# ucsdmanorlab/PSSR2

Hardware: AMD Instinct MI355X
Metric: HR tiles/sec (512^2 4xSR) train (higher is better)
Workload: dtype bf16

## Files before the change

### include/pssr_mi355.h

```cpp
#ifndef PSSR_MI355_H
#define PSSR_MI355_H

#include <stdint.h>

#ifdef __cplusplus
extern "C" {
#endif

typedef void* pssr_stream_t;

enum { PSSR_F32 = 0, PSSR_BF16 = 1, PSSR_F16 = 2 };

enum {
    PSSR_OK = 0,
    PSSR_ERR_ARG = -1,
    PSSR_ERR_LAUNCH = -2,
    PSSR_ERR_UNSUPPORTED = -3
};

int pssr_abi_version(void);
const char* pssr_last_error(void);

int pssr_pack_conv_weight(const float* w_oihw, void* packed, int cout, int cin, int ks,
                          int ci_begin, int ci_count, int mode, const int32_t* n_perm,
// ... 178 lines not shown
int pssr_bilinear_down_u8(const uint8_t* hr, uint8_t* tmp, uint8_t* lr, int planes, int H, int W,
                          int h, int w, pssr_stream_t stream);
int pssr_u8_to_f32(const uint8_t* in, float* out, int64_t n, pssr_stream_t stream);
int pssr_crappify_gaussian(const float* in, float* out, int tiles, int64_t per_tile, float intensity,
                           float gain, float spread, uint64_t seed, uint64_t tile_offset,
                           const double* noise, int flags, const uint64_t* tile_counter,
                           pssr_stream_t stream);
int pssr_crappify_poisson(const float* in, float* out, int tiles, int64_t per_tile, float intensity,
                          float gain, float spread, uint64_t seed, uint64_t tile_offset, int flags,
                          const uint64_t* tile_counter, pssr_stream_t stream);
int pssr_crappify_poisson_samples(const float* in, const double* samples, float* out, int64_t n, double intensity,
                                  double gain, int flags, pssr_stream_t stream);
int pssr_counter_add(uint64_t* counter, uint64_t inc, pssr_stream_t stream);
int pssr_gaussian_blur(const float* in, float* tmp, float* out, int planes, int h, int w, float sigma,
                       float gain, int flags, pssr_stream_t stream);

int pssr_crappify_saltpepper(const float* in, float* out, int tiles, int64_t per_tile, float amount, float gain, float spread,
                             uint64_t seed, uint64_t tile_offset, int flags, const uint64_t* tile_counter, pssr_stream_t stream);
int pssr_gaussian_blur_tiles(const float* in, float* tmp, float* out, int tiles, int planes_per_tile, int h, int w, float sigma,
                             float spread, float gain, uint64_t seed, uint64_t tile_offset, int flags, const uint64_t* tile_counter,
                             pssr_stream_t stream);
typedef struct pssr_gather_item { const uint8_t* src; int sh, sw, rot, flip_axis; } pssr_gather_item;
int pssr_gen_pair_geometry_u8(const pssr_gather_item* items_dev, int n_items, uint8_t* out, int c, int res, pssr_stream_t stream);
typedef struct pssr_sheet_desc { const uint8_t* base; int frames, h, w, reserved; } pssr_sheet_desc;
typedef struct pssr_window_item { int sheet, frame0, y0, x0, rot, flip_axis; } pssr_window_item;
int pssr_gather_windows_u8(const pssr_sheet_desc* sheets_dev, int n_sheets, const pssr_window_item* items_dev, int n_items,
                           uint8_t* out, int c, int res, pssr_stream_t stream);


int pssr_input_plain(const float* x_nchw, void* out, int n, int c, int h, int w, int out_cs, float pre_scale, float pre_shift,
                     int dtype, pssr_stream_t stream);
int pssr_im2col_dil(const void* in, int in_cs, int in_co, int c, const float* scale, const float* shift, void* col, int cp,
                    int n, int h, int w, int dil, int dtype, pssr_stream_t stream);
int pssr_col2im_dil(const void* dcol, int cp, void* out, int out_cs, int out_co, int c, int n, int h, int w, int dil,
                    const void* y, int y_cs, int y_co, const float* scale, const float* shift, const float* mean,
                    const float* invstd, double* stats, int dtype, pssr_stream_t stream);
int pssr_channel_stats_nhwc(const void* x, int cs, int co, int c, int64_t npix, double* stats, int dtype, pssr_stream_t stream);
int pssr_sum_relu(const void* const* ins, const int* in_cs, const int* in_co, int n_in, void* out, int out_cs, int out_co,
                  int64_t npix, int c, int relu, int dtype, pssr_stream_t stream);
int pssr_relu_mask(const void* dout, int do_cs, int do_co, const void* out, int o_cs, int o_co, void* dz, int dz_cs, int dz_co,
                   int64_t npix, int c, int dtype, pssr_stream_t stream);
int pssr_affine_relu(const void* x, int cs, int co, const float* scale, const float* shift, void* out, int out_cs, int out_co,
                     int64_t npix, int c, int dtype, pssr_stream_t stream);
int pssr_maxpool_k(const void* in, int in_cs, int in_co, void* out, int out_cs, int out_co, int n, int h, int w, int c, int k,
                   int dtype, pssr_stream_t stream);
int pssr_maxpool_k_bwd(const void* act, int act_cs, int act_co, const void* dpool, int dp_cs, int dp_co, void* dx, int dx_cs,
// ... 127 lines not shown
```

### pssr2_amd/_lib.py

```python
from __future__ import annotations

import ctypes as C
import os
from pathlib import Path

_LIB_PATH = Path(__file__).resolve().parent / "libpssr_mi355.so"
_lib = None

F32, BF16, F16 = 0, 1, 2
PRO_NONE, PRO_BN_RELU, PRO_GELU = 0, 1, 2
EPI_STORE, EPI_TAIL, EPI_DGRAD_MASK, EPI_FINAL, EPI_DGRAD_GELU, EPI_HEADQ = 0, 1, 2, 3, 4, 5
FLAG_RELU, FLAG_STATS, FLAG_AFFINE, FLAG_HEADQ, FLAG_SHUF2, FLAG_SOLO = 1, 2, 4, 8, 16, 32

c_void_p, c_int, c_i64, c_float = C.c_void_p, C.c_int, C.c_int64, C.c_float


class ConvDesc(C.Structure):
    _fields_ = [
        ("dtype", C.c_int32), ("n", C.c_int32), ("h", C.c_int32), ("w", C.c_int32),
        ("in0", c_void_p), ("in0_cstride", C.c_int32), ("in0_coff", C.c_int32), ("cin0", C.c_int32), ("taps0", C.c_int32),
        ("w0", c_void_p),
        ("in1", c_void_p), ("in1_cstride", C.c_int32), ("in1_coff", C.c_int32), ("cin1", C.c_int32), ("taps1", C.c_int32),
        ("w1", c_void_p),
        ("prologue", C.c_int32), ("pro_scale", c_void_p), ("pro_shift", c_void_p),
# ... 58 lines not shown
                ("mode", C.c_int32), ("k_pad", C.c_int32), ("n_pad", C.c_int32), ("dtype", C.c_int32), ("center", C.c_int32)]


def lib():
    global _lib
    if _lib is None:
        if not _LIB_PATH.exists():
            raise RuntimeError(
                f"{_LIB_PATH} not found: build the HIP extension first (python -c 'import __graft_entry__ as g; g.build()' "
                "or make -C pssr2_amd/csrc). pssr2_amd has no CPU fallback.")
        import torch
        _lib = C.CDLL(str(_LIB_PATH))
        _lib.pssr_last_error.restype = C.c_char_p
        _lib.pssr_packed_weight_bytes.restype = C.c_int64
        _lib.pssr_conv2d_workspace_bytes.restype = C.c_int64
        _lib.pssr_gradhist_workspace_bytes.restype = C.c_int64
        _lib.pssr_noise_profile_workspace_bytes.restype = C.c_int64
        _lib.pssr_noise_profile_workspace_bytes.argtypes = [c_int, c_i64]
        for name in ("pssr_noise_profile_f32", "pssr_noise_profile_u8"):
            getattr(_lib, name).argtypes = [c_void_p, c_void_p, c_void_p, c_void_p, c_int, c_i64, c_void_p, c_i64, c_void_p]
        _lib.pssr_noise_profile_loss.argtypes = [c_void_p, c_void_p, c_void_p, c_void_p, c_int, c_i64, c_int, c_void_p, c_void_p, c_void_p,
                                                 c_void_p]
        _lib.pssr_gather_windows_u8.argtypes = [c_void_p, c_int, c_void_p, c_int, c_void_p, c_int, c_int, c_void_p]
    return _lib


def check(status: int, what: str):
    if status != 0:
        raise RuntimeError(f"{what} failed ({status}): {lib().pssr_last_error().decode()}")


def ptr(t):
    return None if t is None else c_void_p(t.data_ptr())


def stream_ptr():
    import torch
    return c_void_p(torch.cuda.current_stream().cuda_stream)
```

### pssr2_amd/csrc/crappify.hip

```cpp
#include "common.h"

namespace {

constexpr int PRECISION_BITS = 32 - 8 - 2;

struct Taps { int xmin, n; int k[40]; };
__device__ __forceinline__ void pil_taps(int xx, int in_size, int out_size, Taps& t) {
    const double scale = (double)in_size / (double)out_size;
    const double filterscale = scale < 1.0 ? 1.0 : scale;
    const double support = 1.0 * filterscale;
    const double center = (xx + 0.5) * scale;
    const double ss = 1.0 / filterscale;
    int xmin = (int)(center - support + 0.5);
    if (xmin < 0) xmin = 0;
    int xmax = (int)(center + support + 0.5);
    if (xmax > in_size) xmax = in_size;
    const int n = xmax - xmin;
    double w[40];
    double ww = 0.0;
    for (int x = 0; x < n && x < 40; ++x) {
        double a = (x + xmin - center + 0.5) * ss;
        if (a < 0.0) a = -a;
        const double v = a < 1.0 ? 1.0 - a : 0.0;
        w[x] = v; ww += v;
// ... 54 lines not shown
        }
        return make_uint4(c0, c1, c2, c3);
    }
};
__device__ __forceinline__ double u01(uint32_t hi, uint32_t lo) {
    const uint64_t v = (((uint64_t)hi << 32) | lo) >> 11;
    return ((double)v + 0.5) * (1.0 / 9007199254740992.0);
}
__device__ __forceinline__ double normal_from(const uint4& r) {
    const double u1 = u01(r.x, r.y), u2 = u01(r.z, r.w);
    return sqrt(-2.0 * log(u1)) * cos(6.283185307179586476925 * u2);
}
__device__ __forceinline__ double finish(double v, int flags) {
    if (flags & 2) v = rint(v);
    if (flags & 3) v = v < 0.0 ? 0.0 : (v > 255.0 ? 255.0 : v);
    return v;
}
__device__ __forceinline__ double tile_intensity(const Philox& ph, float intensity, float spread) {
    if (!(spread > 0.f)) return intensity;
    const double v = (double)intensity + (double)spread * normal_from(ph(~0ull, 7u));
    return v > 0.0 ? v : 0.0;
}

__global__ void gaussian_noise_kernel(const float* __restrict__ in, float* __restrict__ out, int tiles, long per_tile, float intensity,
                                      float gain, float spread, uint64_t seed, uint64_t tile_offset, const double* __restrict__ noise, int flags,
                                      const uint64_t* __restrict__ tile_counter) {
    if (tile_counter) tile_offset += tile_counter[0];
    const long total = (long)tiles * per_tile;
    for (long i = blockIdx.x * (long)blockDim.x + threadIdx.x; i < total; i += (long)gridDim.x * blockDim.x) {
        const long tile = i / per_tile, pix = i % per_tile;
        double nz;
        if (noise) nz = noise[i];
        else {
            const Philox ph(seed, tile_offset + tile);
            nz = (double)gain + tile_intensity(ph, intensity, spread) * normal_from(ph((uint64_t)pix, 0u));
        }
        out[i] = (float)finish((double)in[i] + nz, flags);
    }
}

__device__ double poisson_draw(const Philox& ph, uint64_t pix, double lam) {
    if (lam <= 0.0) return 0.0;
    uint32_t sub = 1;
    if (lam < 10.0) {
        const double enlam = exp(-lam);
        double prod = 1.0; long x = 0;
        for (int it = 0; it < 64; ++it) {
            const uint4 r = ph(pix, sub++);
            const double u[2] = {u01(r.x, r.y), u01(r.z, r.w)};
            for (int j = 0; j < 2; ++j) { prod *= u[j]; if (prod > enlam) ++x; else return (double)x; }
        }
        return (double)x;
    }
    const double slam = sqrt(lam), loglam = log(lam);
    const double b = 0.931 + 2.53 * slam, a = -0.059 + 0.02483 * b;
    const double invalpha = 1.1239 + 1.1328 / (b - 3.4), vr = 0.9277 - 3.6224 / (b - 2.0);
    for (int it = 0; it < 256; ++it) {
        const uint4 r = ph(pix, sub++);
        const double U = u01(r.x, r.y) - 0.5, V = u01(r.z, r.w);
        const double us = 0.5 - fabs(U);
        const double k = floor((2.0 * a / us + b) * U + lam + 0.43);
        if (us >= 0.07 && V <= vr) return k;
        if (k < 0.0 || (us < 0.013 && V > us)) continue;
        if (log(V) + log(invalpha) - log(a / (us * us) + b) <= -lam + k * loglam - lgamma(k + 1.0)) return k;
    }
    return floor(lam + 0.5);
}

__global__ void poisson_noise_kernel(const float* __restrict__ in, float* __restrict__ out, int tiles, long per_tile, float intensity,
                                     float gain, float spread, uint64_t seed, uint64_t tile_offset, int flags,
                                     const uint64_t* __restrict__ tile_counter) {
    if (tile_counter) tile_offset += tile_counter[0];
    const long total = (long)tiles * per_tile;
    for (long i = blockIdx.x * (long)blockDim.x + threadIdx.x; i < total; i += (long)gridDim.x * blockDim.x) {
        const long tile = i / per_tile, pix = i % per_tile;
        const Philox ph(seed, tile_offset + tile);
        const double x = (double)in[i];
        const double y = poisson_draw(ph, (uint64_t)pix, x > 0.0 ? x : 0.0);
        const double mixv = tile_intensity(ph, intensity, spread);
        out[i] = (float)finish(x * (1.0 - mixv) + y * mixv + (double)gain, flags);
    }
}

__global__ void poisson_samples_kernel(const float* __restrict__ in, const double* __restrict__ samples, float* __restrict__ out, long n,
                                       double intensity, double gain, int flags) {
    const float keep = (float)(1.0 - intensity);
    for (long i = blockIdx.x * (long)blockDim.x + threadIdx.x; i < n; i += (long)gridDim.x * blockDim.x) {
        const float t1 = __fmul_rn(in[i], keep);
        const double v = __dadd_rn(__dadd_rn((double)t1, __dmul_rn(samples[i], intensity)), gain);
        out[i] = (float)finish(v, flags);
    }
}

__global__ void blur_pass_kernel(const float* __restrict__ in, float* __restrict__ out, int planes, int h, int w, float sigma, int axis,
                                 float gain, int flags) {
    const int r = (int)(4.0f * sigma + 0.5f);
    const long total = (long)planes * h * w;
    for (long i = blockIdx.x * (long)blockDim.x + threadIdx.x; i < total; i += (long)gridDim.x * blockDim.x) {
        const int x = i % w, y = (i / w) % h;
        const long base = i - (long)y * w - x;
        double wsum = 0.0, acc = 0.0;
        for (int t = -r; t <= r; ++t) {
            const double wt = exp(-0.5 / ((double)sigma * sigma) * (double)t * t);
// ... 35 lines not shown
        const double sigma = tile_intensity(ph, intensity, spread);
        const int x = i % w, y = (i / w) % h;
        const long base = i - (long)y * w - x;
        double v = (double)in[i];
        if (sigma > 0.0) {
            const int r = (int)(4.0 * (double)(float)sigma + 0.5);
            double wsum = 0.0, acc = 0.0;
            for (int t = -r; t <= r; ++t) {
                const double wt = exp(-0.5 / (sigma * sigma) * (double)t * t);
                int yy = y, xx = x;
                if (axis == 0) { yy = y + t; yy = yy < 0 ? 0 : (yy >= h ? h - 1 : yy); }
                else { xx = x + t; xx = xx < 0 ? 0 : (xx >= w ? w - 1 : xx); }
                wsum += wt; acc += wt * (double)in[base + (long)yy * w + xx];
            }
            v = (double)(float)(acc / wsum);
        }
        if (axis == 1) v = finish((double)(float)v + (double)gain, flags);
        out[i] = (float)v;
    }
}

struct GatherItem { const uint8_t* src; int sh, sw, rot, flip_axis; };

__global__ void gen_pair_geometry_kernel(const GatherItem* __restrict__ items, uint8_t* __restrict__ out, int c, int res) {
    const GatherItem it = items[blockIdx.y];
    const long per_tile = (long)c * res * res;
    const int size = it.sh < it.sw ? (it.sh < res ? it.sh : res) : (it.sw < res ? it.sw : res);
    const bool exact = it.sh == res && it.sw == res;
    const int sx = exact ? 0 : (it.sh - size) / 2, sy = exact ? 0 : (it.sw - size) / 2;
    for (long i = blockIdx.x * (long)blockDim.x + threadIdx.x; i < per_tile; i += (long)gridDim.x * blockDim.x) {
        int ox = (int)(i % res), oy = (int)((i / res) % res), oc = (int)(i / ((long)res * res));
        if (it.flip_axis == 0) oc = c - 1 - oc;
        if (it.flip_axis == 1 || it.flip_axis == 3) oy = res - 1 - oy;
        if (it.flip_axis == 2 || it.flip_axis == 3) ox = res - 1 - ox;
        int py = oy, px = ox;
        if (it.rot) { py = ox; px = res - 1 - oy; }
        if (size > 1) {
            const int period = 2 * (size - 1);
            py %= period; px %= period;
            if (py >= size) py = period - py;
            if (px >= size) px = period - px;
        } else { py = 0; px = 0; }
        out[blockIdx.y * per_tile + i] = it.src[((long)oc * it.sh + sx + py) * it.sw + sy + px];
    }
}

static inline int grid1d(long total) { long b = (total + 255) / 256; return (int)(b < 8192 ? (b > 0 ? b : 1) : 8192); }

}

extern "C" {

int pssr_bilinear_down_u8(const uint8_t* hr, uint8_t* tmp, uint8_t* lr, int planes, int H, int W, int h, int w, pssr_stream_t s) {
    PSSR_CHECK(hr && tmp && lr && planes > 0 && H > 0 && W > 0 && h > 0 && w > 0, PSSR_ERR_ARG, "bilinear_down_u8: bad args");
    PSSR_CHECK(H >= h && W >= w && (double)W / w <= 19.0 && (double)H / h <= 19.0, PSSR_ERR_UNSUPPORTED, "bilinear_down_u8: reduction ratio must be in [1, 19]");
    long rows = (long)planes * H;
    const long row_groups = (rows + 15) / 16;
    hipLaunchKernelGGL(resample_h_kernel, dim3(cdiv(w, 64), (unsigned)(row_groups < 65535 ? row_groups : 65535)), dim3(64), 0, (hipStream_t)s, hr, tmp, planes, H, W, w);
    PSSR_LAUNCH_CHECK();
    hipLaunchKernelGGL(resample_v_kernel, dim3(cdiv(w, 128), h, planes < 1024 ? planes : 1024), dim3(128), 0, (hipStream_t)s, tmp, lr, planes, H, h, w);
    PSSR_LAUNCH_CHECK();
    return PSSR_OK;
}

int pssr_u8_to_f32(const uint8_t* in, float* out, int64_t n, pssr_stream_t s) {
    PSSR_CHECK(in && out && n > 0, PSSR_ERR_ARG, "u8_to_f32: bad args");
    hipLaunchKernelGGL(u8_to_f32_kernel, dim3(grid1d(n)), dim3(256), 0, (hipStream_t)s, in, out, (long)n);
    PSSR_LAUNCH_CHECK();
    return PSSR_OK;
// ... 58 lines not shown
                             float gain, uint64_t seed, uint64_t tile_offset, int flags, const uint64_t* tile_counter, pssr_stream_t s) {
    PSSR_CHECK(in && tmp && out && tiles > 0 && planes_per_tile > 0 && h > 0 && w > 0 && sigma >= 0.f && spread >= 0.f && flags >= 0 && flags <= 3,
               PSSR_ERR_ARG, "gaussian_blur_tiles: bad args");
    const long total = (long)tiles * planes_per_tile * h * w;
    hipLaunchKernelGGL(blur_pass_tiles_kernel, dim3(grid1d(total)), dim3(256), 0, (hipStream_t)s, in, tmp, tiles, planes_per_tile, h, w, sigma,
                       spread, seed, tile_offset, 0, 0.f, 0, tile_counter);
    PSSR_LAUNCH_CHECK();
    hipLaunchKernelGGL(blur_pass_tiles_kernel, dim3(grid1d(total)), dim3(256), 0, (hipStream_t)s, tmp, out, tiles, planes_per_tile, h, w, sigma,
                       spread, seed, tile_offset, 1, gain, flags, tile_counter);
    PSSR_LAUNCH_CHECK();
    return PSSR_OK;
}

int pssr_gen_pair_geometry_u8(const pssr_gather_item* items_dev, int n_items, uint8_t* out, int c, int res, pssr_stream_t s) {
    PSSR_CHECK(items_dev && out && n_items > 0 && n_items <= 65535 && c > 0 && res > 0, PSSR_ERR_ARG, "gen_pair_geometry: bad args");
    static_assert(sizeof(pssr_gather_item) == sizeof(GatherItem), "pssr_gather_item layout");
    const long per_tile = (long)c * res * res;
    long gx = (per_tile + 255) / 256; if (gx > 256) gx = 256;
    hipLaunchKernelGGL(gen_pair_geometry_kernel, dim3((unsigned)gx, n_items), dim3(256), 0, (hipStream_t)s, (const GatherItem*)items_dev, out, c, res);
    PSSR_LAUNCH_CHECK();
    return PSSR_OK;
}

}
```

### pssr2_amd/data.py

```python
from __future__ import annotations

import glob
import random
import warnings
from pathlib import Path

import numpy as np
import torch
from torch.utils.data import Dataset

from .crappifiers import Crappifier, Poisson
from .util import _force_list


def _square_crop(image, max_res):
    h, w = image.shape[-2:]
    if [h, w] == [max_res] * 2:
        return image
    size = min(h, w, max_res)
    sx, sy = (h - size) // 2, (w - size) // 2
    return image[:, sx:sx + size, sy:sy + size]


def _pad_image(image, res):
# ... 552 lines not shown
    def __repr__(self):
        return (f'PairedSlidingDataset from paths "{self.hr_path}" and "{self.lr_path}"\n{len(self.hr_files)} paired files with {len(self)} '
                f"total frame slices\nhigh-res: {self.hr_res}, low-res: {self.hr_res // self.lr_scale}")


def synthetic_em_tile(index, res=512, channels=1):
    rng = np.random.default_rng(1234 + index)
    out = []
    for _ in range(channels):
        white = rng.standard_normal((res, res))
        f = np.fft.rfft2(white)
        ky, kx = np.fft.fftfreq(res)[:, None], np.fft.rfftfreq(res)[None, :]
        smooth = np.fft.irfft2(f * np.exp(-2 * (np.pi * 3.0) ** 2 * (kx ** 2 + ky ** 2)), s=(res, res))
        smooth /= smooth.std() + 1e-12
        out.append(np.clip(128 + 48 * smooth + 8 * rng.standard_normal((res, res)), 0, 255).astype(np.uint8))
    return np.stack(out)


class DevicePairGenerator:

    def __init__(self, lr_scale=4, crappifier=Poisson(), seed=0, tile_counter=None):
        self.lr_scale, self.crappifier, self.seed = lr_scale, crappifier, seed
        self.tile_counter = tile_counter

    def _stage(self, x, spec, seed, tile_offset, flags):
        from . import ops
        kind, intensity, gain, spread = spec
        if kind == "gaussian":
            return ops.crappify_gaussian(x, intensity, gain, spread, seed, tile_offset, flags, tile_counter=self.tile_counter)
        if kind == "poisson":
            return ops.crappify_poisson(x, intensity, gain, spread, seed, tile_offset, flags, tile_counter=self.tile_counter)
        if kind == "blur":
            if spread > 0:
                return ops.gaussian_blur_tiles(x, intensity, spread, gain, seed, tile_offset, flags, tile_counter=self.tile_counter)
            return ops.gaussian_blur(x, intensity, gain, flags)
        if kind == "saltpepper":
            return ops.crappify_saltpepper(x, intensity, gain, spread, seed, tile_offset, flags, tile_counter=self.tile_counter)
        raise NotImplementedError(kind)

    def __call__(self, hr_u8: torch.Tensor, tile_offset: int = 0):
        from . import ops
        if not hr_u8.is_cuda or hr_u8.dtype != torch.uint8:
            raise RuntimeError("DevicePairGenerator needs a uint8 tensor on the MI355X")
        hr_u8 = hr_u8.contiguous()
        b, c, h, w = hr_u8.shape
        lr = ops.u8_to_f32(ops.bilinear_down_u8(hr_u8, h // self.lr_scale, w // self.lr_scale))
        cr = self.crappifier
        if cr is not None:
            spec = cr.device_spec()
            if isinstance(spec, list):
                clip = ops.CLIP if spec[0][0] == "clip" else 0
                stages = spec[1:]
                for i, st in enumerate(stages):
                    last = i == len(stages) - 1
                    lr = self._stage(lr, st, self.seed + 7919 * i, tile_offset, ops.ROUND_CLIP if last and clip else (clip if not last else 0))
                if not clip:
                    lr = self._stage(lr, ("gaussian", 0.0, 0.0, 0.0), 0, 0, ops.ROUND_CLIP)
            else:
                lr = self._stage(lr, spec, self.seed, tile_offset, ops.ROUND_CLIP)
        return ops.u8_to_f32(hr_u8), lr

    def from_stacks(self, stacks, hr_res, rotations=None, tile_offset: int = 0):
        from . import ops
        rotations = [False] * len(stacks) if rotations is None else rotations
        return self(ops.gen_pair_geometry_u8(stacks, rotations, hr_res), tile_offset)


def _gather_table(images, indices, rotations):
    import struct
    c, h, w = images.shape[1:]
    base, stride = images.data_ptr(), c * h * w
    buf = bytearray()
    for i, rot in zip(indices, rotations):
        axis = -1
        if rot:
            axis = 3 if isinstance(rot[1], (tuple, list)) else int(rot[1])
        buf += struct.pack("<Qiiii", base + int(i) * stride, h, w, int(bool(rot and rot[0])), axis)
    if not buf:
        return torch.zeros(0, 3, dtype=torch.int64, device=images.device)
    return torch.frombuffer(buf, dtype=torch.int64).view(-1, 3).to(images.device)


class DeviceTileDataset(Dataset):
# ... 23 lines not shown
        self.names = names if names is not None else [f"image{i}" for i in range(n)]
        self._val_set, self._val_key = set(self.val_idx), None
        self.tile_counter = torch.zeros(1, dtype=torch.int64, device=self.images.device)
        self.gen = DevicePairGenerator(self.lr_scale, crappifier, seed=seed, tile_counter=self.tile_counter)
        self._item_bytes = 24

    def __len__(self):
        return len(self.images)

    def _get_name(self, idx):
        return self.names[idx]

    def _draw_rotation(self, idx):
        key = (id(self.val_idx), len(self.val_idx))
        if key != self._val_key:
            self._val_set, self._val_key = set(self.val_idx), key
        if self.rotation and idx not in self._val_set:
            return [bool(random.getrandbits(1)), random.choice((1, 2, (1, 2)))]
        return False

    def draw_items(self, indices):
        return _gather_table(self.images, indices, [self._draw_rotation(int(i)) for i in indices])

    def device_batch(self, items):
        from . import _lib as L, ops
        b, c = items.shape[0], self.images.shape[1]
        res = self.hr_res // self.lr_scale if self.is_lr else self.hr_res
        out = torch.empty(b, c, res, res, dtype=torch.uint8, device=self.images.device)
        L.check(L.lib().pssr_gen_pair_geometry_u8(L.ptr(items), b, L.ptr(out), c, res, L.stream_ptr()), "pssr_gen_pair_geometry_u8")
        if self.is_lr:
            return ops.u8_to_f32(out)
        hr, lr = self.gen(out)
        ops.counter_add(self.tile_counter, b)
        return hr, lr

    def __getitem__(self, idx):
        if idx >= len(self):
            raise IndexError(f"Tried to retrieve invalid image. Index {idx} is not less than {len(self)} total image frame slices.")
        out = self.device_batch(self.draw_items([idx]))
        return out[0] if self.is_lr else (out[0][0], out[1][0])


class DevicePairedTileDataset(PairedArrayDataset):
    _keep_tensors = True

    def __init__(self, hr_images, lr_images, hr_res=512, lr_scale=4, n_frames=-1, val_split=1, rotation=True, split_seed=None,
                 transforms=None, names=None, device="cuda"):
        if transforms is not None:
            raise NotImplementedError("DevicePairedTileDataset applies no host transforms")
        super().__init__(hr_images, lr_images, hr_res, lr_scale, n_frames, val_split, rotation, split_seed, None, names)
        self.hr_images = torch.as_tensor(self.hr_images).to(device).contiguous()
        self.lr_images = torch.as_tensor(self.lr_images).to(device).contiguous()
        if not self.hr_images.is_cuda:
            raise RuntimeError("DevicePairedTileDataset keeps its images on an MI355X (HIP) device; there is no CPU fallback")
        del self.compact

    def draw_pair_items(self, indices, pp=False):
# ... 79 lines not shown
        self.sheets = self.bank.sheets
        del self.compact
        self.tile_counter = torch.zeros(1, dtype=torch.int64, device=self.bank.device)
        self.gen = DevicePairGenerator(self.lr_scale, crappifier, seed=seed, tile_counter=self.tile_counter)
        self._item_bytes = 24

    def draw_items(self, indices, pp=False):
        entries = []
        for idx in indices:
            idx = int(idx)
            self._check_idx(idx)
            image_idx, local = _get_image_idx(idx, self.slices, self.tiles)
            origin = _window_origin(self.sheets[image_idx], self.hr_res, self.stride, None if self.n_frames is None else self.depth,
                                    self.slices[image_idx], local, self.slide)
            self.bank.check(image_idx, *origin, self.depth, self.hr_res)
            entries.append((image_idx, *origin, self._draw_rotation(idx, pp)))
        return _window_rows(entries).to(self.bank.device)

    def device_batch(self, items):
        from . import ops
        out = self.bank.gather(items, self.depth, self.hr_res)
        if self.is_lr:
            return ops.u8_to_f32(out)
        hr, lr = self.gen(out)
        ops.counter_add(self.tile_counter, items.shape[0])
        nf = self.n_frames
        if nf is not None and nf[0] != nf[1]:
            if not nf[1] > hr.shape[-3]:
                hr = _slice_center(hr, nf[1]).contiguous()
            if not nf[0] > lr.shape[-3]:
                lr = _slice_center(lr, nf[0]).contiguous()
        return hr, lr

    def __getitem__(self, idx, pp=False):
        out = self.device_batch(self.draw_items([idx], pp))
        return out[0] if self.is_lr else (out[0][0], out[1][0])


class DevicePairedSlidingDataset(PairedSlidingArrayDataset):
    _keep_tensors = True

    def __init__(self, hr_sheets, lr_sheets, hr_res=512, lr_scale=4, overlap=128, n_frames=-1, slide=False, val_split=1, rotation=True,
                 split_seed=None, transforms=None, names=None, device="cuda"):
        if transforms is not None:
            raise NotImplementedError("DevicePairedSlidingDataset applies no host transforms")
        super().__init__(hr_sheets, lr_sheets, hr_res, lr_scale, overlap, n_frames, slide, val_split, rotation, split_seed, None, names)
        who, nf = type(self).__name__, self.n_frames
        self.depths = (nf[1], nf[0]) if nf is not None else (_uniform_frames(self.hr_sheets, who), _uniform_frames(self.lr_sheets, who))
# ... 32 lines not shown
```

### pssr2_amd/fastpath.py

```python
from __future__ import annotations

import os

import torch

from . import distributed as D
from .util import SSIMLoss as _SSIMLoss


_CAPTURE_MODE = "thread_local"


def enabled():
    return os.environ.get("PSSR_GRAPH", "1") != "0"


def supports(model, dataset, device):
    if getattr(model, "sync_bn", False) and D.rank_world()[1] > 1:
        return False
    return (enabled() and getattr(model, "_engine", None) is not None and hasattr(dataset, "device_batch") and hasattr(dataset, "draw_items")
            and torch.device(device).type == "cuda" and getattr(dataset, "extra_hr_files", None) is None)


def supports_host(model, dataset, device):
# ... 80 lines not shown
        return self.static


class _Cursor:

    def __init__(self, dataset, batch, capacity, device):
        self.dataset, self.batch = dataset, batch
        self.table = torch.zeros(max(capacity, batch), 3, dtype=torch.int64, device=device)
        self.cursor = torch.zeros(1, dtype=torch.int64, device=device)
        self.ar = torch.arange(batch, device=device)

    def load(self, order):
        rows = self.dataset.draw_items(order)
        if rows.shape[0] > self.table.shape[0]:
            raise RuntimeError("epoch longer than the captured gather table")
        self.table[:rows.shape[0]].copy_(rows)
        self.cursor.zero_()
        return rows.shape[0]

    def next_rows(self):
        rows = self.table[self.ar + self.cursor]
        self.cursor.add_(self.batch)
        return rows

    def tail_rows(self, start, count):
        return self.table[start:start + count]


class TrainStepper:

    WARM = 2

    def __init__(self, model, dataset, batch_size, loss_fn, optim, clamp, image_range, scaler, capacity, device, host=False):
        from .optim import FusedAdamW
        self.model, self.dataset, self.batch, self.loss_fn, self.optim = model, dataset, batch_size, loss_fn, optim
        self.clamp, self.image_range, self.scaler = clamp, image_range, scaler
        self.engine = model._engine
        self.rank, self.world = D.rank_world()
        self.fused = isinstance(optim, FusedAdamW)
        self.amp_dev = scaler is not None and self.fused and self.world == 1 and os.environ.get("PSSR_AMP_DEVICE", "1") != "0"
        self.in_graph_optim = self.fused and self.world == 1 and (scaler is None or self.amp_dev)
        if self.fused:
            optim.device_state = True
        self.scale_dev = (scaler.to_device(device).scale_dev if self.amp_dev else torch.ones(1, device=device)) if scaler is not None else None
        self.host = host
        self.cur = _Cursor(dataset, batch_size, capacity, device) if not host else None
        self.feed = _HostFeed(device) if host else None
        self.device = torch.device(device)
        self.graph, self.outs, self.eager_done = None, None, 0
        self.eager_only = False
        self._reduced = False
        self.split = self.world > 1 and os.environ.get("PSSR_DDP_SPLIT", os.environ.get("PSSR_OVERLAP", "1")) != "0"
        self.graph2, self.split_at = None, 0
        self.comm_events = [] if os.environ.get("PSSR_COMM_STATS") == "1" else None
        self.engine.last_train_stepper = self

    def begin_epoch(self, order):
        self.n = self.cur.load(order)
        self.pos = 0
        return (self.n + self.batch - 1) // self.batch

    def _inputs(self, rows=None):
        if self.host:
            return self.feed.static if rows is None else rows
        return self.dataset.device_batch(self.cur.next_rows() if rows is None else rows)

    def _fwd_bwd(self, rows):
        hr, lr = self._inputs(rows)
        hr_hat = self.model(lr)
        if self.clamp:
            hr_hat = torch.clamp(hr_hat, 0, self.image_range)
        if isinstance(self.loss_fn, _SSIMLoss) and os.environ.get("PSSR_FUSED_DIV", "1") != "0":
            loss = self.loss_fn.forward_divided(hr_hat, hr, self.image_range)
        else:
            loss = self.loss_fn(hr_hat / self.image_range, hr / self.image_range)
        (loss * self.scale_dev if self.scale_dev is not None else loss).backward()
        return hr, lr, hr_hat, loss

    def _body(self, rows=None):
        out = self._fwd_bwd(rows)
        if self.in_graph_optim:
            if self.amp_dev:
                self.scaler.step_dev(self.optim, self.engine._flat_grad)
            else:
                self.optim.step()
            self.optim.zero_grad()
        return out

# ... 191 lines not shown
    def _signature(self):
        m = self.model
        return (self.engine._wepoch[0], tuple(p._version for p in m.parameters()), tuple(b._version for b in m.buffers()))

    def begin(self, order=None):
        if not self.host:
            self.n = self.cur.load(order)
            self.pos = 0
        self.loss_sum.zero_()
        self.count = 0
        if self.weights_move:
            self.engine.mark_weights_changed()
        elif self._signature() != self.sig:
            self.eager_done = 0
        return (self.n + self.batch - 1) // self.batch if not self.host else None

    def _run(self, rows):
        from . import ops
        with torch.no_grad():
            if self.host:
                item = self.feed.static if rows is None else rows
                hr, lr = (None, item[0]) if len(item) == 1 else item
            else:
                item = self.dataset.device_batch(self.cur.next_rows() if rows is None else rows)
                hr, lr = (None, item) if self.dataset.is_lr else item
            hr_hat = self.model(lr)
            if self.clamp:
                hr_hat = torch.clamp(hr_hat, 0, self.image_range)
            loss = None
            if self.loss_fn is not None:
                loss = self.loss_fn(hr_hat / self.image_range, hr / self.image_range)
                self.loss_sum.add_(loss.detach().float().reshape(1))
            u8 = None
            if self.to_u8:
                y = hr_hat.detach().contiguous().float()
                u8 = torch.empty(y.shape, dtype=torch.uint8, device=y.device)
                ops.clip_u8(y, u8)
        return hr, lr, hr_hat, loss, u8

    def step(self, batch=None):
        if self.host:
            batch = tuple(_feedable(t) for t in batch)
            if self.feed.static is None and batch[-1].shape[0] == self.batch:
                self.feed.allocate(batch)
            self.count += 1
            if batch[-1].shape[0] != self.batch or not self.feed.matches(batch):
                if self.weights_move:
# ... 44 lines not shown
```

### pssr2_amd/ops.py

```python
from __future__ import annotations

import ctypes as C

import torch

from . import _lib as L

TORCH_DTYPE = {L.F32: torch.float32, L.BF16: torch.bfloat16, L.F16: torch.float16}


def dtype_code(dt: torch.dtype) -> int:
    if dt == torch.float32:
        return L.F32
    if dt == torch.bfloat16:
        return L.BF16
    if dt == torch.float16:
        return L.F16
    raise ValueError(f"unsupported compute dtype {dt}; use torch.float32, torch.bfloat16 or torch.float16")


def pad_to(v: int, m: int) -> int:
    return (v + m - 1) // m * m


class PackedWeight:
# ... 316 lines not shown

def crappify_poisson_samples(x, samples, intensity, gain, flags, out=None):
    out = torch.empty_like(x) if out is None else out
    if samples.dtype != torch.float64 or samples.numel() != x.numel():
        raise ValueError("samples: float64, one per element of x")
    L.check(L.lib().pssr_crappify_poisson_samples(L.ptr(x), L.ptr(samples.contiguous()), L.ptr(out), C.c_int64(x.numel()), C.c_double(intensity),
                                                  C.c_double(gain), flags, L.stream_ptr()), "pssr_crappify_poisson_samples")
    return out


def gaussian_blur(x, sigma, gain, flags):
    h, w = x.shape[-2:]
    planes = x.numel() // (h * w)
    tmp, out = torch.empty_like(x), torch.empty_like(x)
    L.check(L.lib().pssr_gaussian_blur(L.ptr(x), L.ptr(tmp), L.ptr(out), planes, h, w, C.c_float(sigma), C.c_float(gain), flags,
                                       L.stream_ptr()), "pssr_gaussian_blur")
    return out


def counter_add(counter, inc):
    L.check(L.lib().pssr_counter_add(L.ptr(counter), C.c_uint64(inc), L.stream_ptr()), "pssr_counter_add")


def adamw_step_dev(p, g, m, v, state, beta1, beta2, eps, weight_decay, grad_scale=1.0):
    L.check(L.lib().pssr_adamw_step_dev(L.ptr(p), L.ptr(g), L.ptr(m), L.ptr(v), C.c_int64(p.numel()), L.ptr(state), C.c_float(beta1),
                                        C.c_float(beta2), C.c_float(eps), C.c_float(weight_decay), C.c_float(grad_scale),
                                        L.stream_ptr()), "pssr_adamw_step_dev")


def amp_check(g, amp):
    L.check(L.lib().pssr_amp_check(L.ptr(g), C.c_int64(g.numel()), L.ptr(amp), L.stream_ptr()), "pssr_amp_check")


def adamw_step_amp(p, g, m, v, state, beta1, beta2, eps, weight_decay, amp, growth, backoff, interval, grad_scale=1.0):
    L.check(L.lib().pssr_adamw_step_amp(L.ptr(p), L.ptr(g), L.ptr(m), L.ptr(v), C.c_int64(p.numel()), L.ptr(state), C.c_float(beta1),
                                        C.c_float(beta2), C.c_float(eps), C.c_float(weight_decay), C.c_float(grad_scale), L.ptr(amp),
                                        C.c_float(growth), C.c_float(backoff), int(interval), L.stream_ptr()), "pssr_adamw_step_amp")


def input_patchify(x, xpatch, scale, shift, patch, dtype, pre_scale=1 / 128, pre_shift=-1.0):
    n, c, h, w = x.shape
    L.check(L.lib().pssr_input_patchify(L.ptr(x), L.ptr(xpatch), n, c, h, w, patch, xpatch.shape[-1], C.c_float(pre_scale),
                                        C.c_float(pre_shift), L.ptr(scale), L.ptr(shift), dtype, L.stream_ptr()), "pssr_input_patchify")


def input_norm_bwd2(dxcol_a, dxcol_b, dpatch, patch, x, mean, invstd, stats, dtype, pre_scale=1 / 128, pre_shift=-1.0):
# ... 395 lines not shown
```

Measured before the change: 2602.

## Fuse HR gather, PIL downsample, noise and counter advance into one kernel

Adds a single kernel that gathers each HR tile with its rotation, flip and reflect padding into LDS strips. From there it writes the float HR output, runs the separable PIL-style antialiased downsample, and applies Gaussian or Poisson noise. The cursor row index and tile counter advance happen on the device through a last-block ticket. This replaces the separate passes for geometry, bilinear downsample, u8-to-f32 conversion, crappify, cursor indexing and counter add, cutting launches and intermediate global traffic in the data-pipeline part of each training step. The trade-offs are heavy LDS use and only a few blocks per tile, plus reliance on atomics for cross-block coordination.

New measurement: 2411. -7.3%, worse.

```diff
diff --git a/include/pssr_mi355.h b/include/pssr_mi355.h
--- a/include/pssr_mi355.h
+++ b/include/pssr_mi355.h
@@ -224,6 +224,11 @@
                              pssr_stream_t stream);
 typedef struct pssr_gather_item { const uint8_t* src; int sh, sw, rot, flip_axis; } pssr_gather_item;
 int pssr_gen_pair_geometry_u8(const pssr_gather_item* items_dev, int n_items, uint8_t* out, int c, int res, pssr_stream_t stream);
+int pssr_gen_pair_fused_strip(int res, int scale);
+int pssr_gen_pair_fused_u8(const pssr_gather_item* items_dev, int64_t n_table, const uint8_t* batch, int64_t* cursor,
+                           uint64_t* tile_counter, uint32_t* ticket, int advance, float* hr, float* lr, int b, int c, int res,
+                           int scale, int kind, float intensity, float gain, float spread, uint64_t seed, uint64_t tile_offset,
+                           int flags, pssr_stream_t stream);
 typedef struct pssr_sheet_desc { const uint8_t* base; int frames, h, w, reserved; } pssr_sheet_desc;
 typedef struct pssr_window_item { int sheet, frame0, y0, x0, rot, flip_axis; } pssr_window_item;
 int pssr_gather_windows_u8(const pssr_sheet_desc* sheets_dev, int n_sheets, const pssr_window_item* items_dev, int n_items,
diff --git a/pssr2_amd/_lib.py b/pssr2_amd/_lib.py
--- a/pssr2_amd/_lib.py
+++ b/pssr2_amd/_lib.py
@@ -104,6 +104,9 @@
         _lib.pssr_noise_profile_loss.argtypes = [c_void_p, c_void_p, c_void_p, c_void_p, c_int, c_i64, c_int, c_void_p, c_void_p, c_void_p,
                                                  c_void_p]
         _lib.pssr_gather_windows_u8.argtypes = [c_void_p, c_int, c_void_p, c_int, c_void_p, c_int, c_int, c_void_p]
+        _lib.pssr_gen_pair_fused_strip.argtypes = [c_int, c_int]
+        _lib.pssr_gen_pair_fused_u8.argtypes = [c_void_p, c_i64, c_void_p, c_void_p, c_void_p, c_void_p, c_int, c_void_p, c_void_p, c_int, c_int,
+                                                c_int, c_int, c_int, c_float, c_float, c_float, C.c_uint64, C.c_uint64, c_int, c_void_p]
     return _lib
 
 
diff --git a/pssr2_amd/csrc/crappify.hip b/pssr2_amd/csrc/crappify.hip
--- a/pssr2_amd/csrc/crappify.hip
+++ b/pssr2_amd/csrc/crappify.hip
@@ -100,6 +100,10 @@
     return v > 0.0 ? v : 0.0;
 }
 
+__device__ __forceinline__ double gaussian_nz(const Philox& ph, uint64_t pix, float intensity, float gain, float spread) {
+    return (double)gain + tile_intensity(ph, intensity, spread) * normal_from(ph(pix, 0u));
+}
+
 __global__ void gaussian_noise_kernel(const float* __restrict__ in, float* __restrict__ out, int tiles, long per_tile, float intensity,
                                       float gain, float spread, uint64_t seed, uint64_t tile_offset, const double* __restrict__ noise, int flags,
                                       const uint64_t* __restrict__ tile_counter) {
@@ -111,7 +115,7 @@
         if (noise) nz = noise[i];
         else {
             const Philox ph(seed, tile_offset + tile);
-            nz = (double)gain + tile_intensity(ph, intensity, spread) * normal_from(ph((uint64_t)pix, 0u));
+            nz = gaussian_nz(ph, (uint64_t)pix, intensity, gain, spread);
         }
         out[i] = (float)finish((double)in[i] + nz, flags);
     }
@@ -145,6 +149,12 @@
     return floor(lam + 0.5);
 }
 
+__device__ __forceinline__ double poisson_mix(const Philox& ph, uint64_t pix, double x, float intensity, float gain, float spread) {
+    const double y = poisson_draw(ph, pix, x > 0.0 ? x : 0.0);
+    const double mixv = tile_intensity(ph, intensity, spread);
+    return x * (1.0 - mixv) + y * mixv + (double)gain;
+}
+
 __global__ void poisson_noise_kernel(const float* __restrict__ in, float* __restrict__ out, int tiles, long per_tile, float intensity,
                                      float gain, float spread, uint64_t seed, uint64_t tile_offset, int flags,
                                      const uint64_t* __restrict__ tile_counter) {
@@ -153,10 +163,7 @@
     for (long i = blockIdx.x * (long)blockDim.x + threadIdx.x; i < total; i += (long)gridDim.x * blockDim.x) {
         const long tile = i / per_tile, pix = i % per_tile;
         const Philox ph(seed, tile_offset + tile);
-        const double x = (double)in[i];
-        const double y = poisson_draw(ph, (uint64_t)pix, x > 0.0 ? x : 0.0);
-        const double mixv = tile_intensity(ph, intensity, spread);
-        out[i] = (float)finish(x * (1.0 - mixv) + y * mixv + (double)gain, flags);
+        out[i] = (float)finish(poisson_mix(ph, (uint64_t)pix, (double)in[i], intensity, gain, spread), flags);
     }
 }
 
@@ -238,29 +245,178 @@
 
 struct GatherItem { const uint8_t* src; int sh, sw, rot, flip_axis; };
 
+struct PairGeom { int size, sx, sy; };
+__device__ __forceinline__ PairGeom pair_geom(const GatherItem& it, int res) {
+    PairGeom g;
+    g.size = it.sh < it.sw ? (it.sh < res ? it.sh : res) : (it.sw < res ? it.sw : res);
+    const bool exact = it.sh == res && it.sw == res;
+    g.sx = exact ? 0 : (it.sh - g.size) / 2; g.sy = exact ? 0 : (it.sw - g.size) / 2;
+    return g;
+}
+__device__ __forceinline__ long pair_src_offset(const GatherItem& it, const PairGeom& g, int c, int res, int oc, int oy, int ox) {
+    if (it.flip_axis == 0) oc = c - 1 - oc;
+    if (it.flip_axis == 1 || it.flip_axis == 3) oy = res - 1 - oy;
+    if (it.flip_axis == 2 || it.flip_axis == 3) ox = res - 1 - ox;
+    int py = oy, px = ox;
+    if (it.rot) { py = ox; px = res - 1 - oy; }
+    if (g.size > 1) {
+        if (g.size < res) {
+            const int period = 2 * (g.size - 1);
+            py %= period; px %= period;
+            if (py >= g.size) py = period - py;
+            if (px >= g.size) px = period - px;
+        }
+    } else { py = 0; px = 0; }
+    return ((long)oc * it.sh + g.sx + py) * it.sw + g.sy + px;
+}
+
 __global__ void gen_pair_geometry_kernel(const GatherItem* __restrict__ items, uint8_t* __restrict__ out, int c, int res) {
     const GatherItem it = items[blockIdx.y];
     const long per_tile = (long)c * res * res;
-    const int size = it.sh < it.sw ? (it.sh < res ? it.sh : res) : (it.sw < res ? it.sw : res);
-    const bool exact = it.sh == res && it.sw == res;
-    const int sx = exact ? 0 : (it.sh - size) / 2, sy = exact ? 0 : (it.sw - size) / 2;
+    const PairGeom g = pair_geom(it, res);
     for (long i = blockIdx.x * (long)blockDim.x + threadIdx.x; i < per_tile; i += (long)gridDim.x * blockDim.x) {
-        int ox = (int)(i % res), oy = (int)((i / res) % res), oc = (int)(i / ((long)res * res));
-        if (it.flip_axis == 0) oc = c - 1 - oc;
-        if (it.flip_axis == 1 || it.flip_axis == 3) oy = res - 1 - oy;
-        if (it.flip_axis == 2 || it.flip_axis == 3) ox = res - 1 - ox;
-        int py = oy, px = ox;
-        if (it.rot) { py = ox; px = res - 1 - oy; }
-        if (size > 1) {
-            const int period = 2 * (size - 1);
-            py %= period; px %= period;
-            if (py >= size) py = period - py;
-            if (px >= size) px = period - px;
-        } else { py = 0; px = 0; }
-        out[blockIdx.y * per_tile + i] = it.src[((long)oc * it.sh + sx + py) * it.sw + sy + px];
-    }
-}
-
+        const int ox = (int)(i % res), oy = (int)((i / res) % res), oc = (int)(i / ((long)res * res));
+        out[blockIdx.y * per_tile + i] = it.src[pair_src_offset(it, g, c, res, oc, oy, ox)];
+    }
+}
+
+struct FusedArgs {
+    const GatherItem* items; long n_table;
+    const uint8_t* batch;
+    long long* cursor; unsigned long long* tile_counter; unsigned* ticket; int advance;
+    float* hr; float* lr;
+    int b, c, res, h, strip, kmax, max_rows, pitch, wp;
+    float intensity, gain, spread; uint64_t seed, tile_offset; int flags;
+};
+enum { FUSED_NONE = 0, FUSED_GAUSSIAN = 1, FUSED_POISSON = 2 };
+
+static inline int fused_max_rows(int res, int h, int strip) {
+    const int cs = (res + h - 1) / h;
+    return (strip + 2) * cs + 2 < res ? (strip + 2) * cs + 2 : res;
+}
+static inline int fused_kmax(int res, int h) { const int k = 2 * ((res + h - 1) / h) + 2; return k < 40 ? k : 40; }
+static inline long fused_lds_bytes(int res, int h, int strip) {
+    const int rows = fused_max_rows(res, h, strip), pitch = ((res + 3) & ~3) + 4, wp = (h + 3) & ~3;
+    return (long)(2 + fused_kmax(res, h)) * (h + strip) * 4 + (long)rows * pitch + (long)rows * wp;
+}
+
+template <int KIND> __global__ __launch_bounds__(256) void gen_pair_fused_kernel(const FusedArgs a) {
+    extern __shared__ __attribute__((aligned(16))) char smem[];
+    const int tid = threadIdx.x, res = a.res, h = a.h, w = a.h, S = a.strip, kmax = a.kmax;
+    const int ch = blockIdx.y, item = blockIdx.z, y0 = blockIdx.x * S;
+    int* col_xmin = (int*)smem; int* col_n = col_xmin + w; int* col_k = col_n + w;
+    int* row_xmin = col_k + kmax * w; int* row_n = row_xmin + S; int* row_k = row_n + S;
+    uint8_t* src8 = (uint8_t*)(row_k + kmax * S);
+    uint8_t* tmp8 = src8 + (long)a.max_rows * a.pitch;
+
+    const long long cur = a.cursor ? __hip_atomic_load(a.cursor, __ATOMIC_RELAXED, __HIP_MEMORY_SCOPE_AGENT) : 0;
+    const uint64_t tc = a.tile_counter ? __hip_atomic_load(a.tile_counter, __ATOMIC_RELAXED, __HIP_MEMORY_SCOPE_AGENT) : 0;
+
+    GatherItem it;
+    bool valid = true;
+    if (a.items) {
+        const long long row = cur + item;
+        valid = row >= 0 && row < a.n_table;
+        if (valid) it = a.items[row]; else { it.src = nullptr; it.sh = it.sw = res; it.rot = 0; it.flip_axis = -1; }
+    } else {
+        it.src = a.batch + (long)item * a.c * res * res; it.sh = it.sw = res; it.rot = 0; it.flip_axis = -1;
+    }
+    const PairGeom g = pair_geom(it, res);
+
+    for (int j = tid; j < w + S; j += 256) {
+        Taps t;
+        if (j < w) {
+            pil_taps(j, res, w, t);
+            const int n = t.n < kmax ? t.n : kmax;
+            col_xmin[j] = t.xmin; col_n[j] = n;
+            for (int x = 0; x < n; ++x) col_k[x * w + j] = t.k[x];
+        } else {
+            const int yy = j - w;
+            int n = 0;
+            t.xmin = 0;
+            if (y0 + yy < h) { pil_taps(y0 + yy, res, h, t); n = t.n < kmax ? t.n : kmax; }
+            row_xmin[yy] = t.xmin; row_n[yy] = n;
+            for (int x = 0; x < n; ++x) row_k[x * S + yy] = t.k[x];
+        }
+    }
+    __syncthreads();
+    const int ys = (h - y0 < S ? h - y0 : S) - 1;
+    const int wy0 = row_xmin[0];
+    int nrows = row_xmin[ys] + row_n[ys] - wy0;
+    if (nrows > a.max_rows) nrows = a.max_rows;
+
+    const unsigned total = (unsigned)nrows * (unsigned)res;
+    for (unsigned e = tid; e < total; e += 256) {
+        unsigned r, ox;
+        if (it.rot) { ox = e / (unsigned)nrows; r = e - ox * (unsigned)nrows; }
+        else { r = e / (unsigned)res; ox = e - r * (unsigned)res; }
+        src8[r * a.pitch + ox] = valid ? it.src[pair_src_offset(it, g, a.c, res, ch, wy0 + (int)r, (int)ox)] : (uint8_t)0;
+    }
+    __syncthreads();
+
+    {
+        int r0 = (int)((long)y0 * res / h), r1 = y0 + S >= h ? res : (int)((long)(y0 + S) * res / h);
+        if (r0 < wy0) r0 = wy0;
+        if (r1 > wy0 + nrows) r1 = wy0 + nrows;
+        float* dst = a.hr + (((long)item * a.c + ch) * res + r0) * res;
+        const uint8_t* s8 = src8 + (r0 - wy0) * a.pitch;
+        if ((res & 3) == 0) {
+            const unsigned q = (unsigned)res >> 2, n4 = (unsigned)(r1 - r0) * q;
+            for (unsigned e = tid; e < n4; e += 256) {
+                const unsigned r = e / q, x4 = e - r * q;
+                const uint32_t v = *(const uint32_t*)(s8 + r * a.pitch + 4 * x4);
+                *(float4*)(dst + (long)r * res + 4 * x4) = make_float4((float)(v & 255u), (float)((v >> 8) & 255u), (float)((v >> 16) & 255u), (float)(v >> 24));
+            }
+        } else {
+            const unsigned n1 = (unsigned)(r1 - r0) * (unsigned)res;
+            for (unsigned e = tid; e < n1; e += 256) {
+                const unsigned r = e / (unsigned)res, x = e - r * (unsigned)res;
+                dst[(long)r * res + x] = (float)s8[r * a.pitch + x];
+            }
+        }
+    }
+
+    const unsigned toth = (unsigned)nrows * (unsigned)w;
+    for (unsigned e = tid; e < toth; e += 256) {
+        const unsigned r = e / (unsigned)w, ox = e - r * (unsigned)w;
+        const uint8_t* src = src8 + r * a.pitch + col_xmin[ox];
+        const int n = col_n[ox];
+        int acc = 1 << (PRECISION_BITS - 1);
+        for (int x = 0; x < n; ++x) acc += (int)src[x] * col_k[x * w + ox];
+        tmp8[r * a.wp + ox] = clip8(acc);
+    }
+    __syncthreads();
+
+    const unsigned totv = (unsigned)(ys + 1) * (unsigned)w;
+    for (unsigned e = tid; e < totv; e += 256) {
+        const unsigned yy = e / (unsigned)w, ox = e - yy * (unsigned)w;
+        const int first = row_xmin[yy] - wy0, n = row_n[yy];
+        int acc = 1 << (PRECISION_BITS - 1);
+        for (int y = 0; y < n; ++y)
+            if (first + y < nrows) acc += (int)tmp8[(first + y) * a.wp + ox] * row_k[y * S + yy];
+        const float x = (float)clip8(acc);
+        const long pix = ((long)ch * h + (y0 + (int)yy)) * w + ox;
+        float v = x;
+        if constexpr (KIND != FUSED_NONE) {
+            const Philox ph(a.seed, a.tile_offset + tc + (uint64_t)item);
+            if constexpr (KIND == FUSED_GAUSSIAN) v = (float)finish((double)x + gaussian_nz(ph, (uint64_t)pix, a.intensity, a.gain, a.spread), a.flags);
+            else v = (float)finish(poisson_mix(ph, (uint64_t)pix, (double)x, a.intensity, a.gain, a.spread), a.flags);
+        }
+        a.lr[(long)item * a.c * h * w + pix] = v;
+    }
+
+    if (a.advance) {
+        __syncthreads();
+        if (tid == 0) {
+            const unsigned groups = gridDim.x * gridDim.y * gridDim.z;
+            if (__hip_atomic_fetch_add(a.ticket, 1u, __ATOMIC_RELAXED, __HIP_MEMORY_SCOPE_AGENT) == groups - 1) {
+                if (a.tile_counter) __hip_atomic_fetch_add(a.tile_counter, (unsigned long long)a.b, __ATOMIC_RELAXED, __HIP_MEMORY_SCOPE_AGENT);
+                if (a.cursor) __hip_atomic_fetch_add(a.cursor, (long long)a.b, __ATOMIC_RELAXED, __HIP_MEMORY_SCOPE_AGENT);
+                __hip_atomic_store(a.ticket, 0u, __ATOMIC_RELAXED, __HIP_MEMORY_SCOPE_AGENT);
+            }
+        }
+    }
+}
 static inline int grid1d(long total) { long b = (total + 255) / 256; return (int)(b < 8192 ? (b > 0 ? b : 1) : 8192); }
 
 }
@@ -365,4 +521,41 @@
     return PSSR_OK;
 }
 
-}
+int pssr_gen_pair_fused_strip(int res, int scale) {
+    if (res <= 0 || scale <= 0 || res / scale <= 0) return 0;
+    const int h = res / scale;
+    if ((double)res / h > 19.0) return 0;
+    for (int strip = 8; strip >= 1; strip /= 2)
+        if (fused_lds_bytes(res, h, strip) <= 64 * 1024) return strip;
+    return 0;
+}
+
+int pssr_gen_pair_fused_u8(const pssr_gather_item* items_dev, int64_t n_table, const uint8_t* batch, int64_t* cursor, uint64_t* tile_counter,
+                           uint32_t* ticket, int advance, float* hr, float* lr, int b, int c, int res, int scale, int kind, float intensity,
+                           float gain, float spread, uint64_t seed, uint64_t tile_offset, int flags, pssr_stream_t s) {
+    PSSR_CHECK(((items_dev != nullptr) != (batch != nullptr)) && hr && lr && b > 0 && b <= 65535 && c > 0 && c <= 65535 && res > 0 && scale > 0,
+               PSSR_ERR_ARG, "gen_pair_fused: bad args");
+    PSSR_CHECK(kind >= FUSED_NONE && kind <= FUSED_POISSON && flags >= 0 && flags <= 3, PSSR_ERR_ARG, "gen_pair_fused: bad noise stage");
+    PSSR_CHECK(!items_dev || n_table > 0, PSSR_ERR_ARG, "gen_pair_fused: empty gather table");
+    PSSR_CHECK(items_dev || !cursor, PSSR_ERR_ARG, "gen_pair_fused: a cursor needs a gather table");
+    PSSR_CHECK(!advance || ((tile_counter || cursor) && ticket), PSSR_ERR_ARG, "gen_pair_fused: advancing needs a counter and a ticket");
+    PSSR_CHECK((long)b * c * res * res < (1l << 40), PSSR_ERR_ARG, "gen_pair_fused: batch too large");
+    const int strip = pssr_gen_pair_fused_strip(res, scale);
+    PSSR_CHECK(strip > 0, PSSR_ERR_UNSUPPORTED, "gen_pair_fused: reduction ratio must be in [1, 19] and the strip must fit 64 KiB of LDS");
+    static_assert(sizeof(pssr_gather_item) == sizeof(GatherItem), "pssr_gather_item layout");
+    FusedArgs a;
+    a.items = (const GatherItem*)items_dev; a.n_table = (long)n_table; a.batch = batch;
+    a.cursor = (long long*)cursor; a.tile_counter = (unsigned long long*)tile_counter; a.ticket = ticket; a.advance = advance != 0;
+    a.hr = hr; a.lr = lr; a.b = b; a.c = c; a.res = res; a.h = res / scale; a.strip = strip;
+    a.kmax = fused_kmax(res, a.h); a.max_rows = fused_max_rows(res, a.h, strip); a.pitch = ((res + 3) & ~3) + 4; a.wp = (a.h + 3) & ~3;
+    a.intensity = intensity; a.gain = gain; a.spread = spread; a.seed = seed; a.tile_offset = tile_offset; a.flags = flags;
+    const dim3 grid(cdiv(a.h, strip), c, b);
+    const size_t lds = (size_t)fused_lds_bytes(res, a.h, strip);
+    if (kind == FUSED_GAUSSIAN) hipLaunchKernelGGL(gen_pair_fused_kernel<FUSED_GAUSSIAN>, grid, dim3(256), lds, (hipStream_t)s, a);
+    else if (kind == FUSED_POISSON) hipLaunchKernelGGL(gen_pair_fused_kernel<FUSED_POISSON>, grid, dim3(256), lds, (hipStream_t)s, a);
+    else hipLaunchKernelGGL(gen_pair_fused_kernel<FUSED_NONE>, grid, dim3(256), lds, (hipStream_t)s, a);
+    PSSR_LAUNCH_CHECK();
+    return PSSR_OK;
+}
+
+}
diff --git a/pssr2_amd/data.py b/pssr2_amd/data.py
--- a/pssr2_amd/data.py
+++ b/pssr2_amd/data.py
@@ -598,6 +598,7 @@
     def __init__(self, lr_scale=4, crappifier=Poisson(), seed=0, tile_counter=None):
         self.lr_scale, self.crappifier, self.seed = lr_scale, crappifier, seed
         self.tile_counter = tile_counter
+        self.ticket = None if tile_counter is None else torch.zeros(1, dtype=torch.int32, device=tile_counter.device)
 
     def _stage(self, x, spec, seed, tile_offset, flags):
         from . import ops
@@ -614,12 +615,24 @@
             return ops.crappify_saltpepper(x, intensity, gain, spread, seed, tile_offset, flags, tile_counter=self.tile_counter)
         raise NotImplementedError(kind)
 
-    def __call__(self, hr_u8: torch.Tensor, tile_offset: int = 0):
+    def fused_spec(self, res):
+        from . import ops
+        if not ops.fused_pairs_enabled():
+            return False, None
+        spec = None if self.crappifier is None else self.crappifier.device_spec()
+        return ops.gen_pair_fused_fits(res, self.lr_scale, spec), spec
+
+    def __call__(self, hr_u8: torch.Tensor, tile_offset: int = 0, advance: bool = False):
         from . import ops
         if not hr_u8.is_cuda or hr_u8.dtype != torch.uint8:
             raise RuntimeError("DevicePairGenerator needs a uint8 tensor on the MI355X")
         hr_u8 = hr_u8.contiguous()
         b, c, h, w = hr_u8.shape
+        advance = advance and self.tile_counter is not None
+        fused, spec = self.fused_spec(h) if h == w and b > 0 else (False, None)
+        if fused:
+            return ops.gen_pair_fused_u8(h, self.lr_scale, spec, self.seed, tile_offset, b, c, hr_u8.device, batch=hr_u8,
+                                         tile_counter=self.tile_counter, ticket=self.ticket, advance=advance)
         lr = ops.u8_to_f32(ops.bilinear_down_u8(hr_u8, h // self.lr_scale, w // self.lr_scale))
         cr = self.crappifier
         if cr is not None:
@@ -634,7 +647,10 @@
                     lr = self._stage(lr, ("gaussian", 0.0, 0.0, 0.0), 0, 0, ops.ROUND_CLIP)
             else:
                 lr = self._stage(lr, spec, self.seed, tile_offset, ops.ROUND_CLIP)
-        return ops.u8_to_f32(hr_u8), lr
+        hr = ops.u8_to_f32(hr_u8)
+        if advance:
+            ops.counter_add(self.tile_counter, b)
+        return hr, lr
 
     def from_stacks(self, stacks, hr_res, rotations=None, tile_offset: int = 0):
         from . import ops
@@ -704,17 +720,27 @@
     def draw_items(self, indices):
         return _gather_table(self.images, indices, [self._draw_rotation(int(i)) for i in indices])
 
-    def device_batch(self, items):
+    def fused_pairs(self):
+        return not self.is_lr and self.gen.fused_spec(self.hr_res)[0]
+
+    def device_batch(self, items, cursor=None, count=None):
         from . import _lib as L, ops
-        b, c = items.shape[0], self.images.shape[1]
+        c = self.images.shape[1]
+        if self.fused_pairs():
+            b = items.shape[0] if cursor is None else count
+            return ops.gen_pair_fused_u8(self.hr_res, self.lr_scale, self.gen.fused_spec(self.hr_res)[1], self.gen.seed, 0, b, c,
+                                         self.images.device, table=items, cursor=cursor, tile_counter=self.tile_counter,
+                                         ticket=self.gen.ticket, advance=True)
+        if cursor is not None:
+            items = items[torch.arange(count, device=cursor.device) + cursor]
+            cursor.add_(count)
+        b = items.shape[0]
         res = self.hr_res // self.lr_scale if self.is_lr else self.hr_res
         out = torch.empty(b, c, res, res, dtype=torch.uint8, device=self.images.device)
         L.check(L.lib().pssr_gen_pair_geometry_u8(L.ptr(items), b, L.ptr(out), c, res, L.stream_ptr()), "pssr_gen_pair_geometry_u8")
         if self.is_lr:
             return ops.u8_to_f32(out)
-        hr, lr = self.gen(out)
-        ops.counter_add(self.tile_counter, b)
-        return hr, lr
+        return self.gen(out, advance=True)
 
     def __getitem__(self, idx):
         if idx >= len(self):
@@ -840,8 +866,7 @@
         out = self.bank.gather(items, self.depth, self.hr_res)
         if self.is_lr:
             return ops.u8_to_f32(out)
-        hr, lr = self.gen(out)
-        ops.counter_add(self.tile_counter, items.shape[0])
+        hr, lr = self.gen(out, advance=True)
         nf = self.n_frames
         if nf is not None and nf[0] != nf[1]:
             if not nf[1] > hr.shape[-3]:
diff --git a/pssr2_amd/fastpath.py b/pssr2_amd/fastpath.py
--- a/pssr2_amd/fastpath.py
+++ b/pssr2_amd/fastpath.py
@@ -126,6 +126,11 @@
         rows = self.table[self.ar + self.cursor]
         self.cursor.add_(self.batch)
         return rows
+
+    def next_batch(self):
+        if getattr(self.dataset, "fused_pairs", None) is not None and self.dataset.fused_pairs():
+            return self.dataset.device_batch(self.table, cursor=self.cursor, count=self.batch)
+        return self.dataset.device_batch(self.next_rows())
 
     def tail_rows(self, start, count):
         return self.table[start:start + count]
@@ -167,7 +172,7 @@
     def _inputs(self, rows=None):
         if self.host:
             return self.feed.static if rows is None else rows
-        return self.dataset.device_batch(self.cur.next_rows() if rows is None else rows)
+        return self.cur.next_batch() if rows is None else self.dataset.device_batch(rows)
 
     def _fwd_bwd(self, rows):
         hr, lr = self._inputs(rows)
@@ -405,7 +410,7 @@
                 item = self.feed.static if rows is None else rows
                 hr, lr = (None, item[0]) if len(item) == 1 else item
             else:
-                item = self.dataset.device_batch(self.cur.next_rows() if rows is None else rows)
+                item = self.cur.next_batch() if rows is None else self.dataset.device_batch(rows)
                 hr, lr = (None, item) if self.dataset.is_lr else item
             hr_hat = self.model(lr)
             if self.clamp:
diff --git a/pssr2_amd/ops.py b/pssr2_amd/ops.py
--- a/pssr2_amd/ops.py
+++ b/pssr2_amd/ops.py
@@ -1,6 +1,7 @@
 from __future__ import annotations
 
 import ctypes as C
+import os
 
 import torch
 
@@ -363,6 +364,30 @@
     L.check(L.lib().pssr_counter_add(L.ptr(counter), C.c_uint64(inc), L.stream_ptr()), "pssr_counter_add")
 
 
+FUSED_KINDS = {None: 0, "gaussian": 1, "poisson": 2}
+
+
+def fused_pairs_enabled():
+    return os.environ.get("PSSR_FUSED_PAIRS", "1") != "0"
+
+
+def gen_pair_fused_fits(res, scale, spec):
+    if spec is not None and not (isinstance(spec, tuple) and spec[0] in ("gaussian", "poisson")):
+        return False
+    return L.lib().pssr_gen_pair_fused_strip(int(res), int(scale)) > 0
+
+
+def gen_pair_fused_u8(res, scale, spec, seed, tile_offset, b, c, device, table=None, batch=None, cursor=None, tile_counter=None,
+                      ticket=None, advance=False):
+    kind, intensity, gain, spread = (None, 0.0, 0.0, 0.0) if spec is None else spec
+    hr = torch.empty(b, c, res, res, dtype=torch.float32, device=device)
+    lr = torch.empty(b, c, res // scale, res // scale, dtype=torch.float32, device=device)
+    L.check(L.lib().pssr_gen_pair_fused_u8(L.ptr(table), 0 if table is None else table.shape[0], L.ptr(batch), L.ptr(cursor), L.ptr(tile_counter),
+                                           L.ptr(ticket), int(bool(advance)), L.ptr(hr), L.ptr(lr), b, c, res, scale, FUSED_KINDS[kind],
+                                           intensity, gain, spread, seed, tile_offset, ROUND_CLIP, L.stream_ptr()), "pssr_gen_pair_fused_u8")
+    return hr, lr
+
+
 def adamw_step_dev(p, g, m, v, state, beta1, beta2, eps, weight_decay, grad_scale=1.0):
     L.check(L.lib().pssr_adamw_step_dev(L.ptr(p), L.ptr(g), L.ptr(m), L.ptr(v), C.c_int64(p.numel()), L.ptr(state), C.c_float(beta1),
                                         C.c_float(beta2), C.c_float(eps), C.c_float(weight_decay), C.c_float(grad_scale),
```
